# uta-smile/Adaptive-Graph-Convolutional-Network

Measured on NVIDIA B200. Metric: sgc_ll_train_graphs_per_s, higher is better.
Workload: dtype f32

## Files before the change

adaptive-graph-convolutional-network_b200/_lib.py:

```python
import ctypes
import os

HERE = os.path.dirname(os.path.abspath(__file__))
LIB_PATH = os.path.join(HERE, "libagcn_sm100.so")

AGCN_OK = 0
VARIANT = {"SGC_LL": 0, "SGC_LL_Reslap": 1}
LAPLACIAN = {"reference_literal": 0, "paper": 1}
METRIC_GRAD = {"reference": 0, "full": 1}
ACT = {"linear": 0, "relu": 1}
LOSS = {"sigmoid_ce": 0, "softmax_ce": 1}
ADJ_RULE = {"mean_distance": 0, "cutoff": 1}
NOTIFY_FN = ctypes.CFUNCTYPE(None, ctypes.c_void_p, ctypes.c_int32, ctypes.c_void_p)
OUT_RES_L, OUT_RES_W, OUT_L_ALL, SAVE_FOR_BACKWARD = 1, 2, 4, 8


class AgcnError(RuntimeError):
    pass


class Desc(ctypes.Structure):
    _fields_ = [("F", ctypes.c_int32), ("Fo", ctypes.c_int32), ("K", ctypes.c_int32), ("variant", ctypes.c_int32),
                ("laplacian_mode", ctypes.c_int32), ("metric_grad", ctypes.c_int32), ("activation", ctypes.c_int32),
                ("flags", ctypes.c_uint32)]
# ... 17 lines not shown
    "agcn_profile_enable": (ctypes.c_int, [ctypes.c_int]),
    "agcn_profile_read": (ctypes.c_int, [ctypes.c_char_p, ctypes.c_size_t, ctypes.POINTER(ctypes.c_size_t)]),
    "agcn_profile_timeline": (ctypes.c_int, [ctypes.c_char_p, ctypes.c_size_t, ctypes.POINTER(ctypes.c_size_t)]),
    "agcn_probe_fp32_fma": (ctypes.c_int, [_P, ctypes.c_int32, _P]),
    "agcn_pack_nodes": (ctypes.c_int, [_P, _P, _P, ctypes.c_int32, _P]),
    "agcn_unpack_nodes": (ctypes.c_int, [_P, _P, _P, ctypes.c_int32, _P]),
    "agcn_pack_lap": (ctypes.c_int, [_P, _P, _P, _P]),
    "agcn_capture_begin": (ctypes.c_int, [_P]),
    "agcn_capture_end_launch": (ctypes.c_int, [_P, ctypes.POINTER(ctypes.c_void_p), ctypes.POINTER(ctypes.c_int32)]),
    "agcn_capture_abort": (ctypes.c_int, [_P]),
    "agcn_step_graph_destroy": (ctypes.c_int, [_P]),
    "agcn_unpack_lap": (ctypes.c_int, [_P, _P, _P, _P]),
    "agcn_debug_grouped_product": (ctypes.c_int, [_P, _P, _P, _P, ctypes.c_int32, ctypes.c_int32, ctypes.c_int32,
                                                  ctypes.c_float, ctypes.c_int32, _P]),
    "agcn_debug_grouped_timeline": (ctypes.c_int, [_P]),
    "agcn_pack_lap_csr": (ctypes.c_int, [_P, _P, _P, _P, _P, _P]),
    "agcn_point_laplacian_workspace_bytes": (ctypes.c_int, [_P, ctypes.POINTER(ctypes.c_size_t)]),
    "agcn_point_laplacian": (ctypes.c_int, [_P, _P, ctypes.c_int32, ctypes.c_int32, ctypes.c_float, _P, _P,
                                            ctypes.c_size_t, _P]),
    "agcn_graph_pool": (ctypes.c_int, [_P, _P, _P, _P, _P, ctypes.c_int32, _P]),
    "agcn_graph_pool_backward": (ctypes.c_int, [_P, _P, _P, _P, ctypes.c_int32, _P]),
    "agcn_sgcll_workspace_bytes": (ctypes.c_int, [ctypes.POINTER(Desc), _P, ctypes.POINTER(ctypes.c_size_t),
                                                  ctypes.POINTER(ctypes.c_size_t)]),
    "agcn_sgcll_forward": (ctypes.c_int, [ctypes.POINTER(Desc), _P] + [_P] * 14 + [ctypes.c_size_t, _P]),
    "agcn_sgcll_backward": (ctypes.c_int, [ctypes.POINTER(Desc), _P] + [_P] * 19 + [ctypes.c_size_t, _P]),
    "agcn_gemm_tn_scratch_bytes": (ctypes.c_size_t, [ctypes.c_int32] * 4),
    "agcn_gemm_tn": (ctypes.c_int, [_P, _P, _P, _P, ctypes.c_int32, ctypes.c_int32, ctypes.c_int32, ctypes.c_int32,
                                    _P, ctypes.c_int32, _P]),
    "agcn_node_gemm_scratch_bytes": (ctypes.c_size_t, [ctypes.c_int32, ctypes.c_int32]),
    "agcn_node_gemm": (ctypes.c_int, [_P, ctypes.c_int32, _P, ctypes.c_int32, ctypes.c_int32, _P, ctypes.c_int32,
# ... 70 lines not shown
```

adaptive-graph-convolutional-network_b200/csrc/agcn_head.cu:

```cuda
#include <algorithm>

#include "agcn_internal.cuh"

namespace agcn {

__global__ void segment_sum_kernel(const float* __restrict__ H, const int32_t* __restrict__ node_off, int B, int F,
                                   float* __restrict__ hsum) {
  const int g = blockIdx.x * (blockDim.x >> 5) + (threadIdx.x >> 5), lane = threadIdx.x & 31;
  if (g >= B) return;
  const int r0 = node_off[g], r1 = node_off[g + 1];
  if (F % 32 == 0) {
    for (int c = lane; c < F; c += 32) {
      float s0 = 0.f, s1 = 0.f, s2 = 0.f, s3 = 0.f;
      int r = r0;
      for (; r + 4 <= r1; r += 4) {
        s0 += __ldg(H + (int64_t)r * F + c);
        s1 += __ldg(H + (int64_t)(r + 1) * F + c);
        s2 += __ldg(H + (int64_t)(r + 2) * F + c);
        s3 += __ldg(H + (int64_t)(r + 3) * F + c);
      }
      for (; r < r1; ++r) s0 += __ldg(H + (int64_t)r * F + c);
      hsum[(int64_t)g * F + c] = (s0 + s1) + (s2 + s3);
    }
    return;
// ... 26 lines not shown
  pre[e] = 4.f * ex / ((1.f + ex) * (1.f + ex));
}

__global__ void tanh_bwd_kernel(const float* __restrict__ dtanh, float* __restrict__ dmol, int64_t total) {
  const int64_t e = (int64_t)blockIdx.x * blockDim.x + threadIdx.x;
  if (e >= total) return;
  dmol[e] = dmol[e] * dtanh[e];
}

__global__ void __launch_bounds__(256) weighted_colsum_kernel(const float* __restrict__ M, int ld, int rows, int cols,
                                                              const int32_t* __restrict__ w, float* __restrict__ out) {
  __shared__ float red[8][33];
  const int lane = threadIdx.x & 31, wid = threadIdx.x >> 5;
  const int c = blockIdx.x * 32 + lane;
  float s = 0.f;
  if (c < cols)
    for (int r = wid; r < rows; r += 8) s += (w ? (float)w[r] : 1.f) * M[(int64_t)r * ld + c];
  red[wid][lane] = s;
  __syncthreads();
  if (wid == 0 && c < cols) {
    float t = 0.f;
#pragma unroll
    for (int k = 0; k < 8; ++k) t += red[k][lane];
    out[c] = t;
  }
}

__global__ void segment_broadcast_kernel(const float* __restrict__ dhsum, const int32_t* __restrict__ node_off, int B,
                                         int F, float* __restrict__ dH) {
  const int g = blockIdx.x * (blockDim.x >> 5) + (threadIdx.x >> 5), lane = threadIdx.x & 31;
  if (g >= B) return;
  const int r0 = node_off[g], r1 = node_off[g + 1];
  for (int c = lane; c < F; c += 32) {
    const float v = dhsum[(int64_t)g * F + c];
    for (int r = r0; r < r1; ++r) dH[(int64_t)r * F + c] = v;
  }
}

__global__ void copy_pitched_kernel(const float* __restrict__ src, int lds, float* __restrict__ dst, int ldd, int rows,
                                    int cols) {
  const int64_t e = (int64_t)blockIdx.x * blockDim.x + threadIdx.x;
  if (e >= (int64_t)rows * cols) return;
  const int r = (int)(e / cols), c = (int)(e % cols);
  dst[(int64_t)r * ldd + c] = src[(int64_t)r * lds + c];
}

__global__ void softmax_ce_kernel(float* __restrict__ logits, int ld, const float* __restrict__ y, const float* __restrict__ w,
                                  int B, int C, float scale, float* __restrict__ part) {
  const int b = blockIdx.x * (blockDim.x >> 5) + (threadIdx.x >> 5), lane = threadIdx.x & 31;
  if (b >= B) return;
  float* x = logits + (int64_t)b * ld;
  const float* yb = y + (int64_t)b * C;
  float mx = -INFINITY;
  for (int c = lane; c < C; c += 32) mx = fmaxf(mx, x[c]);
#pragma unroll
  for (int o = 16; o > 0; o >>= 1) mx = fmaxf(mx, __shfl_xor_sync(0xffffffffu, mx, o));
  float se = 0.f, sy = 0.f, sxy = 0.f;
  for (int c = lane; c < C; c += 32) {
    se += expf(x[c] - mx);
// ... 25 lines not shown
}

namespace {

int tn_any(const GemmTNArgs& t, cudaStream_t st) {
  if (tc_gemm_tn_supported(t)) return tc_gemm_tn(t, st);
  return gemm_tn(t, st);
}
size_t tn_any_partial(const GemmTNArgs& t) {
  return std::max(tc_gemm_tn_partial_floats(t), gemm_tn_partial_floats(t.M, t.Kd, t.N, t.S));
}

inline size_t al256(size_t x) { return (x + 255) & ~(size_t)255; }
inline int pad4(int x) { return (x + 3) & ~3; }

struct HeadWork {
  float *hsum, *pre, *mol, *dlog, *dmol, *dhsum, *dWh_pad, *loss_part, *tcA, *tcB, *tcC, *tcD, *tn_part, *splitk;
  size_t bytes;
};

HeadWork carve_head(const agcn_plan* plan, int Fh, int Fm, int Nt, void* base) {
  char* b = reinterpret_cast<char*>(base);
  size_t off = 0;
  auto take = [&](size_t floats) {
    float* r = b ? reinterpret_cast<float*>(b + off) : nullptr;
    off += al256(floats * sizeof(float));
    return r;
  };
  const size_t B = plan->B;
  const int Ntp = pad4(Nt);
  HeadWork w{};
  w.hsum = take(B * Fh);
// ... 5 lines not shown
  w.dWh_pad = take((size_t)Fm * Ntp);
  GemmArgs g;
  g.M = (int)B; g.N = Nt; g.Z = 1;
  w.loss_part = take(std::max((size_t)tc_gemm_loss_parts(g), B) + 64);
  w.tcA = take(tc_gemm_scratch_floats(Fm, Fh, 1, 1));
  w.tcB = take(tc_gemm_scratch_floats(Nt, Fm, 1, 1));
  w.tcC = take(tc_gemm_scratch_floats(Fm, Nt, 1, 1));
  w.tcD = take(tc_gemm_scratch_floats(Fh, Fm, 1, 1));
  GemmTNArgs t;
  t.M = (int)B; t.Kd = std::min(Fm, 128); t.N = Ntp; t.S = 1;
  size_t tn = tn_any_partial(t);
  t.Kd = Fh; t.N = Fm;
  tn = std::max(tn, tn_any_partial(t));
  w.tn_part = take(tn);
  w.splitk = take((size_t)8 * B * std::max(Fm, Fh));
  w.bytes = off;
  return w;
}

}
}

using namespace agcn;

extern "C" {

int agcn_expand_labels(const uint8_t* y, const float* w, int32_t B, int32_t n_tasks, float* d_targets, float* d_weights,
                       void* stream) {
  AGCN_REQUIRE(y && w && d_targets && d_weights && B >= 1 && n_tasks >= 1, "expand_labels: bad arguments");
  AGCN_REQUIRE((reinterpret_cast<uintptr_t>(d_targets) & 7) == 0 && (reinterpret_cast<uintptr_t>(d_weights) & 7) == 0,
               "expand_labels: outputs must be 8-byte aligned");
  const long long n = (long long)B * n_tasks;
  const unsigned grid = (unsigned)std::max<long long>(1, std::min<long long>((n + 1023) / 1024, 8));
  expand_labels_kernel<<<grid, 1024, 0, (cudaStream_t)stream>>>(y, w, n, reinterpret_cast<float2*>(d_targets),
                                                               reinterpret_cast<float2*>(d_weights));
  AGCN_LAUNCH_CHECK();
  return AGCN_OK;
}

int agcn_head_workspace_bytes(const agcn_plan* plan, int32_t Fh, int32_t Fm, int32_t Nt, size_t* bytes) {
  AGCN_REQUIRE(plan && bytes && Fh >= 1 && Fm >= 1 && Nt >= 1, "head_workspace_bytes: bad arguments");
  *bytes = carve_head(plan, Fh, Fm, Nt, nullptr).bytes + 256;
  return AGCN_OK;
}

int agcn_head_loss_grad(const agcn_plan* plan, const float* d_H, const float* d_dense_W, const float* d_dense_b,
                        const float* d_head_W, const float* d_head_b, const float* d_targets, const float* d_weights,
                        float scale, int32_t Fh, int32_t Fm, int32_t Nt, float* d_loss, float* d_dH,
                        float* d_ddense_W, float* d_ddense_b, float* d_dhead_W, float* d_dhead_b, void* d_work,
                        size_t work_bytes, void* stream) {
  return agcn_head_loss_grad_ex(plan, d_H, d_dense_W, d_dense_b, d_head_W, d_head_b, d_targets, d_weights, scale,
                                AGCN_LOSS_SIGMOID_CE, Fh, Fm, Nt, d_loss, d_dH, d_ddense_W, d_ddense_b, d_dhead_W,
                                d_dhead_b, d_work, work_bytes, stream);
}

int agcn_head_loss_grad_ex(const agcn_plan* plan, const float* d_H, const float* d_dense_W, const float* d_dense_b,
                           const float* d_head_W, const float* d_head_b, const float* d_targets, const float* d_weights,
                           float scale, int32_t loss_kind, int32_t Fh, int32_t Fm, int32_t Nt, float* d_loss,
                           float* d_dH, float* d_ddense_W, float* d_ddense_b, float* d_dhead_W, float* d_dhead_b,
                           void* d_work, size_t work_bytes, void* stream) {
  AGCN_REQUIRE(plan && d_H && d_dense_W && d_dense_b && d_head_W && d_head_b && d_targets && d_weights && d_loss &&
                   d_dH && d_ddense_W && d_ddense_b && d_dhead_W && d_dhead_b && d_work,
               "head_loss_grad: null pointer");
  AGCN_REQUIRE(loss_kind == AGCN_LOSS_SIGMOID_CE || loss_kind == AGCN_LOSS_SOFTMAX_CE, "head_loss_grad: unknown loss_kind");
  AGCN_REQUIRE(Fh >= 1 && Fm >= 32 && Fm % 4 == 0 && Nt >= 1,
               "head_loss_grad: unsupported sizes (need Fm >= 32 and a multiple of 4)");
  cudaStream_t st = (cudaStream_t)stream;
  int rc = plan_use(plan, st);
  if (rc) return rc;
  HeadWork w = carve_head(plan, Fh, Fm, Nt, d_work);
  if (w.bytes > work_bytes) {
    set_error("head_loss_grad: workspace too small");
    return AGCN_ERR_WORKSPACE;
  }
  const int B = plan->B, Ntp = pad4(Nt);
  const int R = (int)plan->R;
  (void)R;
  cudaStream_t side = plan->side;

  GemmArgs g_pre, g_log, g_dmol, g_dhs;
  g_pre.M = B; g_pre.N = Fm; g_pre.Kd = Fh;
  g_pre.A0 = w.hsum; g_pre.lda0 = Fh;
  g_pre.B = d_dense_W; g_pre.ldb = Fm;
  g_pre.C = w.pre; g_pre.ldc = Fm;
  g_log.M = B; g_log.N = Nt; g_log.Kd = Fm;
  g_log.A0 = w.mol; g_log.lda0 = Fm;
  g_log.B = d_head_W; g_log.ldb = Nt;
  g_log.C = w.dlog; g_log.ldc = Ntp;
  g_log.bias = d_head_b;
  const bool sigmoid = loss_kind == AGCN_LOSS_SIGMOID_CE;
  if (sigmoid) {
    g_log.bce_y = d_targets; g_log.bce_w = d_weights; g_log.bce_ld = Nt; g_log.bce_scale = scale;
    g_log.loss_part = w.loss_part;
  }
  g_dmol.M = B; g_dmol.N = Fm; g_dmol.Kd = Nt;
  g_dmol.A0 = w.dlog; g_dmol.lda0 = Ntp;
  g_dmol.B = d_head_W; g_dmol.ldb = Nt; g_dmol.transB = 1;
  g_dmol.C = w.dmol; g_dmol.ldc = Fm; g_dmol.split_k_partial = w.splitk;
  g_dhs.M = B; g_dhs.N = Fh; g_dhs.Kd = Fm;
  g_dhs.A0 = w.dmol; g_dhs.lda0 = Fm;
  g_dhs.B = d_dense_W; g_dhs.ldb = Fm; g_dhs.transB = 1;
  g_dhs.C = w.dhsum; g_dhs.ldc = Fh; g_dhs.split_k_partial = w.splitk;
  AGCN_REQUIRE(tc_gemm_supported(g_log), "head_loss_grad: operands are not TMA-compatible (alignment)");
  const bool tc_pre = false, tc_dmol = tc_gemm_supported(g_dmol), tc_dhs = tc_gemm_supported(g_dhs) && (int64_t)B * Fh * Fm > (1ll << 26);
  auto gemm_any = [&](const GemmArgs& g, const float* scratch, bool tc) { return tc ? tc_gemm(g, scratch, st) : gemm_rows(g, st); };
  AGCN_CUDA(cudaEventRecord(plan->ev_side_fork, st));
  AGCN_CUDA(cudaStreamWaitEvent(side, plan->ev_side_fork, 0));
  if (tc_pre && (rc = tc_gemm_split_b(g_pre, w.tcA, side))) return rc;
  if ((rc = tc_gemm_split_b(g_log, w.tcB, side))) return rc;
  if (tc_dmol && (rc = tc_gemm_split_b(g_dmol, w.tcC, side))) return rc;
  if (tc_dhs && (rc = tc_gemm_split_b(g_dhs, w.tcD, side))) return rc;
  if ((rc = zero_async(w.dlog, (size_t)B * Ntp, side))) return rc;
  AGCN_CUDA(cudaEventRecord(plan->ev_side_join, side));

  segment_sum_kernel<<<(B + 7) / 8, 256, 0, st>>>(d_H, plan->d_node_off, B, Fh, w.hsum);
  AGCN_LAUNCH_CHECK();
  AGCN_CUDA(cudaStreamWaitEvent(st, plan->ev_side_join, 0));
  if ((rc = gemm_any(g_pre, w.tcA, tc_pre))) return rc;
  {
    const int64_t total = (int64_t)B * Fm;
    gather_tanh_kernel<<<(unsigned)((total + 255) / 256), 256, 0, st>>>(w.pre, d_dense_b, plan->d_n, B, Fm, w.mol);
    AGCN_LAUNCH_CHECK();
  }
  if ((rc = tc_gemm(g_log, w.tcB, st))) return rc;
  int n_parts = tc_gemm_loss_parts(g_log);
  if (!sigmoid) {
    softmax_ce_kernel<<<(B + 7) / 8, 256, 0, st>>>(w.dlog, Ntp, d_targets, d_weights, B, Nt, scale, w.loss_part);
    AGCN_LAUNCH_CHECK();
    n_parts = B;
  }
  sum_parts_kernel<<<1, 256, 0, st>>>(w.loss_part, n_parts, d_loss);
  AGCN_LAUNCH_CHECK();

  AGCN_CUDA(cudaEventRecord(plan->ev_side_fork, st));
  AGCN_CUDA(cudaStreamWaitEvent(side, plan->ev_side_fork, 0));
  weighted_colsum_kernel<<<(Nt + 31) / 32, 256, 0, side>>>(w.dlog, Ntp, B, Nt, nullptr, d_dhead_b);
  AGCN_LAUNCH_CHECK();
  for (int f0 = 0; f0 < Fm; f0 += 128) {
    GemmTNArgs t;
    t.M = B; t.Kd = std::min(128, Fm - f0); t.N = Ntp; t.S = 1;
    t.A0 = w.mol + f0; t.lda0 = Fm;
    t.D = w.dlog; t.ldd = Ntp;
    t.out = w.dWh_pad + (size_t)f0 * Ntp; t.partial = w.tn_part;
    if ((rc = tn_any(t, side))) return rc;
  }
  {
    const int64_t total = (int64_t)Fm * Nt;
    copy_pitched_kernel<<<(unsigned)((total + 255) / 256), 256, 0, side>>>(w.dWh_pad, Ntp, d_dhead_W, Nt, Fm, Nt);
    AGCN_LAUNCH_CHECK();
  }

  if ((rc = gemm_any(g_dmol, w.tcC, tc_dmol))) return rc;
  {
    const int64_t total = (int64_t)B * Fm;
    tanh_bwd_kernel<<<(unsigned)((total + 255) / 256), 256, 0, st>>>(w.pre, w.dmol, total);
    AGCN_LAUNCH_CHECK();
  }
  if ((rc = gemm_any(g_dhs, w.tcD, tc_dhs))) return rc;
  segment_broadcast_kernel<<<(B + 7) / 8, 256, 0, st>>>(w.dhsum, plan->d_node_off, B, Fh, d_dH);
  AGCN_LAUNCH_CHECK();
  AGCN_CUDA(cudaEventRecord(plan->ev_fork, st));
  AGCN_CUDA(cudaStreamWaitEvent(side, plan->ev_fork, 0));
  weighted_colsum_kernel<<<(Fm + 31) / 32, 256, 0, side>>>(w.dmol, Fm, B, Fm, plan->d_n, d_ddense_b);
  AGCN_LAUNCH_CHECK();
  {
    GemmTNArgs t;
    t.M = B; t.Kd = Fh; t.N = Fm; t.S = 1;
    t.A0 = w.hsum; t.lda0 = Fh;
    t.D = w.dmol; t.ldd = Fm;
    t.out = d_ddense_W; t.partial = w.tn_part;
    if ((rc = tn_any(t, side))) return rc;
  }
  AGCN_CUDA(cudaEventRecord(plan->ev_side_join, side));
  AGCN_CUDA(cudaStreamWaitEvent(st, plan->ev_side_join, 0));
  return AGCN_OK;
}

}
```

adaptive-graph-convolutional-network_b200/csrc/agcn_internal.cuh:

```cuda
#pragma once
#include <cuda_runtime.h>
#include <stdint.h>

#include <atomic>
#include <string>
#include <vector>

#include "agcn_sgcll.h"

#define AGCN_SMALL_MAX 144
#define AGCN_CHEB_SMALL_MAX 144
#define AGCN_FUSE_MAX_N 64
#define AGCN_FUSE_LCAP 8320
#define AGCN_MID_TILED_MIN 32
#define AGCN_DEGREE_FLOOR 8.271806125530277e-25f

namespace agcn {

#ifdef __CUDACC__
__device__ __forceinline__ float tf32_rn(float x) {
  uint32_t r;
  asm("cvt.rna.tf32.f32 %0, %1;\n" : "=r"(r) : "f"(x));
  return __uint_as_float(r);
}
// ... 118 lines not shown
  int64_t sliceB = 0;
  int transB = 0;
  float* C = nullptr;
  int ldc = 0;
  int64_t sliceC = 0;
  const float* bias = nullptr;
  const float* scale = nullptr;
  int act = AGCN_ACT_LINEAR;
  int accumulate = 0;
  const float* bce_y = nullptr;
  const float* bce_w = nullptr;
  int bce_ld = 0;
  float bce_scale = 1.f;
  float* loss_part = nullptr;
  float* split_k_partial = nullptr;
};
int tc_gemm_loss_parts(const GemmArgs& a);
int gemm_rows(const GemmArgs& a, cudaStream_t st);
bool tc_gemm_supported(const GemmArgs& a);
size_t tc_gemm_scratch_floats(int N, int Kd, int S, int Z);
int tc_gemm_split_b(const GemmArgs& a, float* scratch, cudaStream_t st);
int tc_gemm(const GemmArgs& a, const float* scratch, cudaStream_t st);

struct GemmTNArgs {
  int M = 0;
  int Kd = 0;
  int N = 0;
  int S = 1;
  const float* A0 = nullptr;
  int lda0 = 0;
  const float* A1 = nullptr;
  int lda1 = 0;
  int64_t sliceA1 = 0;
  const float* D = nullptr;
  int ldd = 0;
  float* out = nullptr;
  float* partial = nullptr;
// ... 106 lines not shown
                        cudaStream_t st_small, cudaStream_t st_mid);

class ProfScope {
 public:
  ProfScope(const char* name, cudaStream_t st);
  ~ProfScope();
  ProfScope(const ProfScope&) = delete;
  ProfScope& operator=(const ProfScope&) = delete;

 private:
  const char* name_;
  cudaStream_t st_;
  cudaEvent_t e0_;
};

int zero_async(float* dst, size_t floats, cudaStream_t st);
int plan_use(const agcn_plan* plan, cudaStream_t st);
int fork_streams(const agcn_plan* plan, cudaStream_t main, int n_aux);
int join_streams(const agcn_plan* plan, cudaStream_t main, int n_aux);

}
```

adaptive-graph-convolutional-network_b200/csrc/agcn_stack.cu:

```cuda
#include <algorithm>
#include <cmath>
#include <vector>

#include "agcn_internal.cuh"

struct agcn_stack {
  std::vector<agcn_sgcll_desc> layers;
  int32_t Fm = 0, Nt = 0, loss_kind = 0;
  std::vector<int64_t> off;
};

namespace agcn {

__global__ void __launch_bounds__(256) adam_kernel(float* __restrict__ p, const float* __restrict__ g, float* __restrict__ m,
                                                   float* __restrict__ v, const int32_t* __restrict__ step, long long n,
                                                   float lr, float beta1, float beta2, float eps) {
  __shared__ float s_lr_t;
  if (threadIdx.x == 0) {
    const double t = (double)(*step + 1);
    s_lr_t = (float)((double)lr * sqrt(1.0 - pow((double)beta2, t)) / (1.0 - pow((double)beta1, t)));
  }
  __syncthreads();
  const float lr_t = s_lr_t;
  for (long long i = (long long)blockIdx.x * blockDim.x + threadIdx.x; i < n; i += (long long)gridDim.x * blockDim.x) {
// ... 109 lines not shown
    return AGCN_ERR_WORKSPACE;
  }
  const int nl = (int)s->layers.size();
  auto P = [&](int l, int k) { return s->off[5 * (size_t)l + k] >= 0 ? d_params + s->off[5 * (size_t)l + k] : nullptr; };
  auto G = [&](int l, int k) { return s->off[5 * (size_t)l + k] >= 0 ? d_grads + s->off[5 * (size_t)l + k] : nullptr; };
  const int64_t* ho = &s->off[5 * (size_t)nl];
  const float* x = d_X;
  for (int l = 0; l < nl; ++l) {
    const agcn_sgcll_desc& d = s->layers[l];
    rc = agcn_sgcll_forward(&d, plan, x, d_Lint, nullptr, P(l, 2), P(l, 0), P(l, 1), P(l, 3), nullptr, w.H[l], nullptr,
                            nullptr, nullptr, w.saved[l], w.layer_work, w.layer_work_bytes, stream);
    if (rc) return rc;
    x = w.H[l];
  }
  const agcn_sgcll_desc& last = s->layers[nl - 1];
  rc = agcn_head_loss_grad_ex(plan, w.H[nl - 1], d_params + ho[0], d_params + ho[1], d_params + ho[2], d_params + ho[3],
                              d_targets, d_weights, scale, s->loss_kind, last.Fo, s->Fm, s->Nt, d_loss, w.dA,
                              d_grads + ho[0], d_grads + ho[1], d_grads + ho[2], d_grads + ho[3], w.head_work,
                              w.head_work_bytes, stream);
  if (rc) return rc;
  if (notify) notify(notify_user, nl, stream);
  float* dcur = w.dA;
  float* dnext = w.dB;
  for (int l = nl - 1; l >= 0; --l) {
    const agcn_sgcll_desc& d = s->layers[l];
    const bool full = d.laplacian_mode == AGCN_LAP_PAPER && d.metric_grad == AGCN_METRIC_GRAD_FULL;
    float* dX = (l > 0 || full) ? dnext : nullptr;
    rc = agcn_sgcll_backward(&d, plan, l == 0 ? d_X : w.H[l - 1], d_Lint, nullptr, P(l, 2), P(l, 0), P(l, 3), nullptr,
                             w.H[l], dcur, nullptr, w.saved[l], dX, G(l, 2), G(l, 0), G(l, 1), G(l, 3), nullptr, nullptr,
                             w.layer_work, w.layer_work_bytes, stream);
    if (rc) return rc;
    if (notify) notify(notify_user, l, stream);
    std::swap(dcur, dnext);
  }
// ... 104 lines not shown
```

adaptive-graph-convolutional-network_b200/csrc/agcn_tc_gemm.cu:

```cuda
#include <cuda.h>
#include <cstdio>

#include <algorithm>
#include <cstdlib>
#include <mutex>

#include "agcn_internal.cuh"

namespace agcn {

namespace tc {

constexpr int BM = 128;
constexpr int BK = 32;
constexpr int UMMA_K = 8;
constexpr int A_TILE_BYTES = BM * BK * 4;

__device__ __forceinline__ uint32_t smem_u32(const void* p) { return (uint32_t)__cvta_generic_to_shared(p); }

__device__ __forceinline__ void mbar_init(uint64_t* bar, uint32_t count) {
  asm volatile("mbarrier.init.shared::cta.b64 [%0], %1;\n" ::"r"(smem_u32(bar)), "r"(count) : "memory");
}
__device__ __forceinline__ void mbar_expect_tx(uint64_t* bar, uint32_t bytes) {
  asm volatile("mbarrier.arrive.expect_tx.shared::cta.b64 _, [%0], %1;\n" ::"r"(smem_u32(bar)), "r"(bytes) : "memory");
// ... 577 lines not shown
  return true;
}

static bool tc_gemm_narrow2(const GemmArgs& a) {
  const int Npad = tc_npad(a.N);
  if (!a.bce_y || Npad <= 64) return false;
  const int tiles128 = ((a.M + tc::BM - 1) / tc::BM) * a.Z * (Npad / 128);
  return tiles128 < 148;
}

int tc_gemm_loss_parts(const GemmArgs& a) {
  const int Npad = tc_npad(a.N), BN = (Npad <= 64 || tc_gemm_narrow2(a)) ? 64 : 128;
  return 4 * ((a.M + tc::BM - 1) / tc::BM) * a.Z * (Npad / BN);
}

size_t tc_gemm_scratch_floats(int N, int Kd, int S, int Z) { return 2 * (size_t)Z * S * tc_npad(N) * tc_kpitch(Kd); }

int tc_gemm_split_b(const GemmArgs& a, float* scratch, cudaStream_t st) {
  using namespace tc;
  const long long sn = a.transB ? a.ldb : 1, sk = a.transB ? 1 : a.ldb, ss = a.sliceB;
  const int Npad = tc_npad(a.N), Kp = tc_kpitch(a.Kd);
  const int slices = a.Z * a.S;
  float* Bhi = scratch;
  float* Blo = scratch + (size_t)slices * Npad * Kp;
  const long long total = (long long)slices * Npad * Kp;
  const int blocks = (int)std::min<long long>((total + 255) / 256, 1184);
  split_b_kernel<<<blocks, 256, 0, st>>>(a.B, sn, sk, ss, a.N, Npad, a.Kd, Kp, slices, Bhi, Blo);
  AGCN_LAUNCH_CHECK();
  return AGCN_OK;
}
// ... 10 lines not shown
  const int rows_slice1 = a.S > 1 ? (int)(a.sliceA1 / a.lda1) : 0;
  if (a.S > 1) {
    if ((rc = make_map(&mA1, a.A1, (uint64_t)(a.S - 2) * rows_slice1 + a.M, (uint64_t)a.Kd, (uint64_t)a.lda1, BM)))
      return rc;
  } else {
    mA1 = mA0;
  }
  const bool narrow2 = tc_gemm_narrow2(a);
  const int BN = (Npad <= 64 || narrow2) ? 64 : 128;
  if ((rc = make_map(&mBhi, Bhi, (uint64_t)slices * Npad, (uint64_t)a.Kd, (uint64_t)Kp, BN))) return rc;
  if ((rc = make_map(&mBlo, Blo, (uint64_t)slices * Npad, (uint64_t)a.Kd, (uint64_t)Kp, BN))) return rc;
  Args p;
  p.M = a.M; p.N = a.N; p.Kd = a.Kd; p.S = a.S;
  p.kb_per_slice = (a.Kd + BK - 1) / BK;
  const int total_kb = a.S * p.kb_per_slice;
  const int out_tiles = ((a.M + BM - 1) / BM) * a.Z * (Npad / BN);
  int ksplit = 1;
  if (a.split_k_partial && !a.bias && !a.scale && a.act == AGCN_ACT_LINEAR && !a.accumulate && !a.bce_y && a.ldc == a.N && a.Z == 1 &&
      total_kb >= 16 && out_tiles < 74)
    ksplit = std::min(std::min(8, total_kb / 4), std::max(1, 148 / out_tiles));
  p.ksplit = ksplit;
  p.kb_per_split = (total_kb + ksplit - 1) / ksplit;
  p.ksplit = (total_kb + p.kb_per_split - 1) / p.kb_per_split;
  ksplit = p.ksplit;
  p.rows_slice1 = rows_slice1;
  p.b_rows_slice = Npad;
  p.C = a.C; p.ldc = a.ldc; p.sliceC = a.sliceC;
  if (ksplit > 1) {
    p.C = a.split_k_partial;
    p.sliceC = (long long)a.M * a.ldc;
  }
  p.bias = a.bias; p.scale = a.scale; p.act = a.act; p.accumulate = a.accumulate;
  p.bce_y = a.bce_y; p.bce_w = a.bce_w; p.bce_scale = a.bce_scale; p.loss_part = a.loss_part;
  p.bce_ld = a.bce_ld > 0 ? a.bce_ld : a.ldc;
  dim3 grid((a.M + BM - 1) / BM, a.Z * ksplit, Npad / BN);
  static std::once_flag once64, once128;
  if (narrow2) {
    static std::once_flag once642;
    std::call_once(once642, [] {
// ... 9 lines not shown
    });
    {
      ProfScope prof("tc::tc_gemm_kernel", st);
      tc_gemm_kernel<64><<<grid, 192, Smem<64>::TOTAL, st>>>(mA0, mA1, mBhi, mBlo, p);
    }
  } else {
    std::call_once(once128, [] {
      cudaFuncSetAttribute(tc_gemm_kernel<128>, cudaFuncAttributeMaxDynamicSharedMemorySize, Smem<128>::TOTAL);
    });
    {
      ProfScope prof("tc::tc_gemm_kernel", st);
      tc_gemm_kernel<128><<<grid, 192, Smem<128>::TOTAL, st>>>(mA0, mA1, mBhi, mBlo, p);
    }
  }
  AGCN_LAUNCH_CHECK();
  if (ksplit > 1) {
    const long long elems = (long long)a.M * a.ldc;
    reduce_chunks_kernel<<<(unsigned)((elems + 255) / 256), 256, 0, st>>>(a.split_k_partial, a.C, elems, ksplit);
    AGCN_LAUNCH_CHECK();
  }
  return AGCN_OK;
}

}

namespace agcn {

bool tc_gemm_tn_supported(const GemmTNArgs& a) {
  if (ab_env("AGCN_DISABLE_TCGEN05") || ab_env("AGCN_DISABLE_TCGEN05_TN")) return false;
  auto al16 = [](const void* p) { return (reinterpret_cast<uintptr_t>(p) & 15) == 0; };
  if (a.M < 32 || a.Kd > 128 || a.Kd % 4 != 0 || a.N % 4 != 0) return false;
// ... 77 lines not shown
```

include/agcn_sgcll.h:

```cpp
#ifndef AGCN_SGCLL_H_
#define AGCN_SGCLL_H_

#include <stdint.h>
#include <stddef.h>

#ifdef __cplusplus
extern "C" {
#endif

#define AGCN_OK 0
#define AGCN_ERR_INVALID (-1)
#define AGCN_ERR_CUDA (-2)
#define AGCN_ERR_WORKSPACE (-3)
#define AGCN_ERR_NO_DEVICE (-4)

#define AGCN_VARIANT_SGC_LL 0
#define AGCN_VARIANT_SGC_LL_RESLAP 1
#define AGCN_LAP_REFERENCE_LITERAL 0
#define AGCN_LAP_PAPER 1
#define AGCN_METRIC_GRAD_REFERENCE 0
#define AGCN_METRIC_GRAD_FULL 1
#define AGCN_ACT_LINEAR 0
#define AGCN_ACT_RELU 1

// ... 32 lines not shown
int agcn_fused_profile(int enable);
int agcn_fused_profile_read(float* ms_sum, int* launches);

int agcn_profile_enable(int enable);
int agcn_profile_read(char* buf, size_t cap, size_t* needed);
int agcn_profile_timeline(char* buf, size_t cap, size_t* needed);
int agcn_probe_fp32_fma(float* d_sink, int32_t iters, void* stream);

int agcn_fused_debug_set(void* d_buf);

int agcn_debug_grouped_product(const agcn_plan* plan, const float* d_L , const float* d_In ,
                               float* d_Out , int32_t F, int32_t transL, int32_t add_identity, float cmul,
                               int32_t impl, void* stream);

int agcn_debug_grouped_timeline(void* d_buf);

int agcn_pack_nodes(const agcn_plan* plan, const float* d_padded , float* d_packed ,
                    int32_t F, void* stream);
int agcn_unpack_nodes(const agcn_plan* plan, const float* d_packed, float* d_padded, int32_t F, void* stream);
int agcn_pack_lap(const agcn_plan* plan, const float* d_padded , float* d_packed, void* stream);
int agcn_unpack_lap(const agcn_plan* plan, const float* d_packed, float* d_padded, void* stream);
int agcn_pack_lap_csr(const agcn_plan* plan, const int32_t* d_indptr, const int32_t* d_indices, const float* d_values,
                      float* d_packed, void* stream);

#define AGCN_ADJ_MEAN_DISTANCE 0
#define AGCN_ADJ_CUTOFF 1
int agcn_point_laplacian_workspace_bytes(const agcn_plan* plan, size_t* bytes);
int agcn_point_laplacian(const agcn_plan* plan, const float* d_points, int32_t F, int32_t rule, float sparse_ratio,
                         float* d_L, void* d_work, size_t work_bytes, void* stream);

// ... 81 lines not shown
```

Measured before the change: 1.648 million.

## Fuse head segment-sum, dense GEMM and tanh into gather kernels with deferred split-k

Adds fused head kernels. The forward kernel does the per-graph segment sum, the dense projection and tanh plus its derivative in one pass. The backward kernel does the split-k reduction, the tanh backward, the dH-sum GEMM against a transposed weight and the broadcast to nodes. The goal is fewer kernel launches and fewer intermediate round trips through global memory in the small-batch head. It also moves sum_parts to the side stream and adds a weight transpose on that stream. The cost is that the GEMMs run on CUDA cores instead of tensor cores, with a shared-memory limit guard and an env or debug switch to fall back to the old path.

```diff
diff --git a/adaptive-graph-convolutional-network_b200/_lib.py b/adaptive-graph-convolutional-network_b200/_lib.py
--- a/adaptive-graph-convolutional-network_b200/_lib.py
+++ b/adaptive-graph-convolutional-network_b200/_lib.py
@@ -55,6 +55,7 @@
     "agcn_debug_grouped_product": (ctypes.c_int, [_P, _P, _P, _P, ctypes.c_int32, ctypes.c_int32, ctypes.c_int32,
                                                   ctypes.c_float, ctypes.c_int32, _P]),
     "agcn_debug_grouped_timeline": (ctypes.c_int, [_P]),
+    "agcn_debug_head_path": (ctypes.c_int, [ctypes.c_int32]),
     "agcn_pack_lap_csr": (ctypes.c_int, [_P, _P, _P, _P, _P, _P]),
     "agcn_point_laplacian_workspace_bytes": (ctypes.c_int, [_P, ctypes.POINTER(ctypes.c_size_t)]),
     "agcn_point_laplacian": (ctypes.c_int, [_P, _P, ctypes.c_int32, ctypes.c_int32, ctypes.c_float, _P, _P,
diff --git a/adaptive-graph-convolutional-network_b200/csrc/agcn_head.cu b/adaptive-graph-convolutional-network_b200/csrc/agcn_head.cu
--- a/adaptive-graph-convolutional-network_b200/csrc/agcn_head.cu
+++ b/adaptive-graph-convolutional-network_b200/csrc/agcn_head.cu
@@ -1,4 +1,5 @@
 #include <algorithm>
+#include <atomic>
 
 #include "agcn_internal.cuh"
 
@@ -64,8 +65,10 @@
   const int lane = threadIdx.x & 31, wid = threadIdx.x >> 5;
   const int c = blockIdx.x * 32 + lane;
   float s = 0.f;
-  if (c < cols)
+  if (c < cols) {
+#pragma unroll 8
     for (int r = wid; r < rows; r += 8) s += (w ? (float)w[r] : 1.f) * M[(int64_t)r * ld + c];
+  }
   red[wid][lane] = s;
   __syncthreads();
   if (wid == 0 && c < cols) {
@@ -87,12 +90,132 @@
   }
 }
 
+__global__ void transpose_kernel(const float* __restrict__ src, int rows, int cols, float* __restrict__ dst) {
+  const int64_t e = (int64_t)blockIdx.x * blockDim.x + threadIdx.x;
+  if (e >= (int64_t)rows * cols) return;
+  const int r = (int)(e / cols), c = (int)(e % cols);
+  dst[(int64_t)c * rows + r] = src[e];
+}
+
 __global__ void copy_pitched_kernel(const float* __restrict__ src, int lds, float* __restrict__ dst, int ldd, int rows,
                                     int cols) {
   const int64_t e = (int64_t)blockIdx.x * blockDim.x + threadIdx.x;
   if (e >= (int64_t)rows * cols) return;
   const int r = (int)(e / cols), c = (int)(e % cols);
   dst[(int64_t)r * ldd + c] = src[(int64_t)r * lds + c];
+}
+
+constexpr int HEAD_G = 8;
+constexpr int HEAD_KC = 16;
+
+
+__global__ void __launch_bounds__(256) head_gather_fwd_kernel(const float* __restrict__ H, const int32_t* __restrict__ node_off,
+                                                              const int32_t* __restrict__ n_nodes, const float* __restrict__ Wd,
+                                                              const float* __restrict__ bd, int B, int Fh, int Fm, int G,
+                                                              float* __restrict__ hsum, float* __restrict__ dtanh,
+                                                              float* __restrict__ mol) {
+  extern __shared__ __align__(16) float hs[];
+  const int g0 = blockIdx.x * G, ng = min(G, B - g0);
+  for (int e = threadIdx.x; e < ng * Fh; e += blockDim.x) {
+    const int gi = e / Fh, c = e - gi * Fh;
+    const int r0 = node_off[g0 + gi], r1 = node_off[g0 + gi + 1];
+    float v;
+    if (Fh % 32 == 0) {
+      float s0 = 0.f, s1 = 0.f, s2 = 0.f, s3 = 0.f;
+      int r = r0;
+      for (; r + 4 <= r1; r += 4) {
+        s0 += __ldg(H + (int64_t)r * Fh + c);
+        s1 += __ldg(H + (int64_t)(r + 1) * Fh + c);
+        s2 += __ldg(H + (int64_t)(r + 2) * Fh + c);
+        s3 += __ldg(H + (int64_t)(r + 3) * Fh + c);
+      }
+      for (; r < r1; ++r) s0 += __ldg(H + (int64_t)r * Fh + c);
+      v = (s0 + s1) + (s2 + s3);
+    } else {
+      v = 0.f;
+      for (int r = r0; r < r1; ++r) v += H[(int64_t)r * Fh + c];
+    }
+    hs[e] = v;
+    hsum[(int64_t)g0 * Fh + e] = v;
+  }
+  __syncthreads();
+  for (int j = threadIdx.x; j < Fm; j += blockDim.x) {
+    float acc[HEAD_G];
+#pragma unroll
+    for (int gi = 0; gi < HEAD_G; ++gi) acc[gi] = 0.f;
+    for (int k = 0; k < Fh; k += 4) {
+      const float w0 = __ldg(Wd + (int64_t)k * Fm + j), w1 = __ldg(Wd + (int64_t)(k + 1) * Fm + j);
+      const float w2 = __ldg(Wd + (int64_t)(k + 2) * Fm + j), w3 = __ldg(Wd + (int64_t)(k + 3) * Fm + j);
+#pragma unroll
+      for (int gi = 0; gi < HEAD_G; ++gi)
+        if (gi < ng) {
+          const float4 a = *reinterpret_cast<const float4*>(hs + gi * Fh + k);
+          acc[gi] += a.x * w0 + a.y * w1 + a.z * w2 + a.w * w3;
+        }
+    }
+    const float bj = bd[j];
+#pragma unroll
+    for (int gi = 0; gi < HEAD_G; ++gi) {
+      if (gi >= ng) break;
+      const int64_t e = (int64_t)(g0 + gi) * Fm + j;
+      const float a = acc[gi] + (float)n_nodes[g0 + gi] * bj;
+      mol[e] = tanhf(a);
+      const float ex = expf(-2.f * fabsf(a));
+      dtanh[e] = 4.f * ex / ((1.f + ex) * (1.f + ex));
+    }
+  }
+}
+
+__global__ void __launch_bounds__(256) head_gather_bwd_kernel(const float* dmol, int nsplit, int64_t split_stride,
+                                                              const float* __restrict__ dtanh, const float* __restrict__ WdT,
+                                                              const int32_t* __restrict__ node_off, int B, int Fh, int Fm,
+                                                              int G, float* dpre, float* __restrict__ dH) {
+  extern __shared__ __align__(16) float sm[];
+  const int g0 = blockIdx.x * G, ng = min(G, B - g0);
+  float* dp = sm;
+  float* dhs = sm + ng * Fm;
+  for (int e = threadIdx.x; e < ng * Fm; e += blockDim.x) {
+    const int64_t idx = (int64_t)g0 * Fm + e;
+    float s = 0.f;
+    for (int z = 0; z < nsplit; ++z) s += dmol[z * split_stride + idx];
+    const float v = s * dtanh[idx];
+    dp[e] = v;
+    dpre[idx] = v;
+  }
+  __syncthreads();
+  float* ws = dhs + ng * Fh;
+  float acc[8];
+#pragma unroll
+  for (int i = 0; i < 8; ++i) acc[i] = 0.f;
+  for (int k0 = 0; k0 < Fm; k0 += HEAD_KC) {
+    const int kc = min(HEAD_KC, Fm - k0);
+    __syncthreads();
+    for (int e = threadIdx.x; e < kc * Fh; e += blockDim.x) ws[e] = __ldg(WdT + (int64_t)k0 * Fh + e);
+    __syncthreads();
+#pragma unroll
+    for (int i = 0; i < 8; ++i) {
+      const int e = threadIdx.x + i * blockDim.x;
+      if (e < ng * Fh) {
+        const int gi = e / Fh, c = e - gi * Fh;
+        for (int k = 0; k < kc; k += 4) {
+          const float4 a = *reinterpret_cast<const float4*>(dp + gi * Fm + k0 + k);
+          acc[i] += a.x * ws[k * Fh + c] + a.y * ws[(k + 1) * Fh + c] + a.z * ws[(k + 2) * Fh + c] +
+                    a.w * ws[(k + 3) * Fh + c];
+        }
+      }
+    }
+  }
+#pragma unroll
+  for (int i = 0; i < 8; ++i) {
+    const int e = threadIdx.x + i * blockDim.x;
+    if (e < ng * Fh) dhs[e] = acc[i];
+  }
+  __syncthreads();
+  for (int gi = 0; gi < ng; ++gi) {
+    const int r0 = node_off[g0 + gi], r1 = node_off[g0 + gi + 1];
+    float* out = dH + (int64_t)r0 * Fh;
+    for (int e = threadIdx.x; e < (r1 - r0) * Fh; e += blockDim.x) out[e] = dhs[gi * Fh + e % Fh];
+  }
 }
 
 __global__ void softmax_ce_kernel(float* __restrict__ logits, int ld, const float* __restrict__ y, const float* __restrict__ w,
@@ -148,8 +271,20 @@
 inline size_t al256(size_t x) { return (x + 255) & ~(size_t)255; }
 inline int pad4(int x) { return (x + 3) & ~3; }
 
+std::atomic<int> g_head_unfused{0};
+
+inline int head_graphs_per_cta(int B) { return std::min(HEAD_G, std::max(1, (B + 147) / 148)); }
+
+bool head_fused(int B, int Fh, int Fm) {
+  if (g_head_unfused.load(std::memory_order_relaxed) || ab_env("AGCN_HEAD_UNFUSED")) return false;
+  if (Fh % 4 != 0 || Fh > 256) return false;
+  const size_t G = (size_t)head_graphs_per_cta(B);
+  return (G * (Fm + Fh) + HEAD_KC * Fh) * sizeof(float) <= 48 * 1024;
+}
+
 struct HeadWork {
   float *hsum, *pre, *mol, *dlog, *dmol, *dhsum, *dWh_pad, *loss_part, *tcA, *tcB, *tcC, *tcD, *tn_part, *splitk;
+  float* dense_WT;
   size_t bytes;
 };
 
@@ -185,58 +320,24 @@
   tn = std::max(tn, tn_any_partial(t));
   w.tn_part = take(tn);
   w.splitk = take((size_t)8 * B * std::max(Fm, Fh));
+  w.dense_WT = take((size_t)Fh * Fm);
   w.bytes = off;
   return w;
 }
 
 }
-}
-
-using namespace agcn;
-
-extern "C" {
-
-int agcn_expand_labels(const uint8_t* y, const float* w, int32_t B, int32_t n_tasks, float* d_targets, float* d_weights,
-                       void* stream) {
-  AGCN_REQUIRE(y && w && d_targets && d_weights && B >= 1 && n_tasks >= 1, "expand_labels: bad arguments");
-  AGCN_REQUIRE((reinterpret_cast<uintptr_t>(d_targets) & 7) == 0 && (reinterpret_cast<uintptr_t>(d_weights) & 7) == 0,
-               "expand_labels: outputs must be 8-byte aligned");
-  const long long n = (long long)B * n_tasks;
-  const unsigned grid = (unsigned)std::max<long long>(1, std::min<long long>((n + 1023) / 1024, 8));
-  expand_labels_kernel<<<grid, 1024, 0, (cudaStream_t)stream>>>(y, w, n, reinterpret_cast<float2*>(d_targets),
-                                                               reinterpret_cast<float2*>(d_weights));
-  AGCN_LAUNCH_CHECK();
-  return AGCN_OK;
-}
-
-int agcn_head_workspace_bytes(const agcn_plan* plan, int32_t Fh, int32_t Fm, int32_t Nt, size_t* bytes) {
-  AGCN_REQUIRE(plan && bytes && Fh >= 1 && Fm >= 1 && Nt >= 1, "head_workspace_bytes: bad arguments");
-  *bytes = carve_head(plan, Fh, Fm, Nt, nullptr).bytes + 256;
-  return AGCN_OK;
-}
-
-int agcn_head_loss_grad(const agcn_plan* plan, const float* d_H, const float* d_dense_W, const float* d_dense_b,
-                        const float* d_head_W, const float* d_head_b, const float* d_targets, const float* d_weights,
-                        float scale, int32_t Fh, int32_t Fm, int32_t Nt, float* d_loss, float* d_dH,
-                        float* d_ddense_W, float* d_ddense_b, float* d_dhead_W, float* d_dhead_b, void* d_work,
-                        size_t work_bytes, void* stream) {
-  return agcn_head_loss_grad_ex(plan, d_H, d_dense_W, d_dense_b, d_head_W, d_head_b, d_targets, d_weights, scale,
-                                AGCN_LOSS_SIGMOID_CE, Fh, Fm, Nt, d_loss, d_dH, d_ddense_W, d_ddense_b, d_dhead_W,
-                                d_dhead_b, d_work, work_bytes, stream);
-}
-
-int agcn_head_loss_grad_ex(const agcn_plan* plan, const float* d_H, const float* d_dense_W, const float* d_dense_b,
-                           const float* d_head_W, const float* d_head_b, const float* d_targets, const float* d_weights,
-                           float scale, int32_t loss_kind, int32_t Fh, int32_t Fm, int32_t Nt, float* d_loss,
-                           float* d_dH, float* d_ddense_W, float* d_ddense_b, float* d_dhead_W, float* d_dhead_b,
-                           void* d_work, size_t work_bytes, void* stream) {
+
+int head_loss_grad(const agcn_plan* plan, const float* d_H, const float* d_dense_W, const float* d_dense_b,
+                   const float* d_head_W, const float* d_head_b, const float* d_targets, const float* d_weights, float scale,
+                   int32_t loss_kind, int32_t Fh, int32_t Fm, int32_t Nt, float* d_loss, float* d_dH, float* d_ddense_W,
+                   float* d_ddense_b, float* d_dhead_W, float* d_dhead_b, void* d_work, size_t work_bytes, bool join,
+                   cudaStream_t st) {
   AGCN_REQUIRE(plan && d_H && d_dense_W && d_dense_b && d_head_W && d_head_b && d_targets && d_weights && d_loss &&
                    d_dH && d_ddense_W && d_ddense_b && d_dhead_W && d_dhead_b && d_work,
                "head_loss_grad: null pointer");
   AGCN_REQUIRE(loss_kind == AGCN_LOSS_SIGMOID_CE || loss_kind == AGCN_LOSS_SOFTMAX_CE, "head_loss_grad: unknown loss_kind");
   AGCN_REQUIRE(Fh >= 1 && Fm >= 32 && Fm % 4 == 0 && Nt >= 1,
                "head_loss_grad: unsupported sizes (need Fm >= 32 and a multiple of 4)");
-  cudaStream_t st = (cudaStream_t)stream;
   int rc = plan_use(plan, st);
   if (rc) return rc;
   HeadWork w = carve_head(plan, Fh, Fm, Nt, d_work);
@@ -245,9 +346,9 @@
     return AGCN_ERR_WORKSPACE;
   }
   const int B = plan->B, Ntp = pad4(Nt);
-  const int R = (int)plan->R;
-  (void)R;
   cudaStream_t side = plan->side;
+  const bool fused = head_fused(B, Fh, Fm);
+  const int G = head_graphs_per_cta(B), n_cta = (B + G - 1) / G;
 
   GemmArgs g_pre, g_log, g_dmol, g_dhs;
   g_pre.M = B; g_pre.N = Fm; g_pre.Kd = Fh;
@@ -268,12 +369,14 @@
   g_dmol.A0 = w.dlog; g_dmol.lda0 = Ntp;
   g_dmol.B = d_head_W; g_dmol.ldb = Nt; g_dmol.transB = 1;
   g_dmol.C = w.dmol; g_dmol.ldc = Fm; g_dmol.split_k_partial = w.splitk;
+  g_dmol.split_k_defer = fused ? 1 : 0;
   g_dhs.M = B; g_dhs.N = Fh; g_dhs.Kd = Fm;
   g_dhs.A0 = w.dmol; g_dhs.lda0 = Fm;
   g_dhs.B = d_dense_W; g_dhs.ldb = Fm; g_dhs.transB = 1;
   g_dhs.C = w.dhsum; g_dhs.ldc = Fh; g_dhs.split_k_partial = w.splitk;
   AGCN_REQUIRE(tc_gemm_supported(g_log), "head_loss_grad: operands are not TMA-compatible (alignment)");
-  const bool tc_pre = false, tc_dmol = tc_gemm_supported(g_dmol), tc_dhs = tc_gemm_supported(g_dhs) && (int64_t)B * Fh * Fm > (1ll << 26);
+  const bool tc_pre = false, tc_dmol = tc_gemm_supported(g_dmol);
+  const bool tc_dhs = !fused && tc_gemm_supported(g_dhs) && (int64_t)B * Fh * Fm > (1ll << 26);
   auto gemm_any = [&](const GemmArgs& g, const float* scratch, bool tc) { return tc ? tc_gemm(g, scratch, st) : gemm_rows(g, st); };
   AGCN_CUDA(cudaEventRecord(plan->ev_side_fork, st));
   AGCN_CUDA(cudaStreamWaitEvent(side, plan->ev_side_fork, 0));
@@ -282,30 +385,58 @@
   if (tc_dmol && (rc = tc_gemm_split_b(g_dmol, w.tcC, side))) return rc;
   if (tc_dhs && (rc = tc_gemm_split_b(g_dhs, w.tcD, side))) return rc;
   if ((rc = zero_async(w.dlog, (size_t)B * Ntp, side))) return rc;
+  if (fused) {
+    const int64_t total = (int64_t)Fh * Fm;
+    transpose_kernel<<<(unsigned)((total + 255) / 256), 256, 0, side>>>(d_dense_W, Fh, Fm, w.dense_WT);
+    AGCN_LAUNCH_CHECK();
+  }
   AGCN_CUDA(cudaEventRecord(plan->ev_side_join, side));
 
-  segment_sum_kernel<<<(B + 7) / 8, 256, 0, st>>>(d_H, plan->d_node_off, B, Fh, w.hsum);
-  AGCN_LAUNCH_CHECK();
-  AGCN_CUDA(cudaStreamWaitEvent(st, plan->ev_side_join, 0));
-  if ((rc = gemm_any(g_pre, w.tcA, tc_pre))) return rc;
-  {
+  if (fused) {
+    {
+      ProfScope prof("head::head_gather_fwd_kernel", st);
+      head_gather_fwd_kernel<<<n_cta, 256, (size_t)G * Fh * sizeof(float), st>>>(
+          d_H, plan->d_node_off, plan->d_n, d_dense_W, d_dense_b, B, Fh, Fm, G, w.hsum, w.pre, w.mol);
+    }
+    AGCN_LAUNCH_CHECK();
+    AGCN_CUDA(cudaStreamWaitEvent(st, plan->ev_side_join, 0));
+  } else {
+    {
+      ProfScope prof("head::segment_sum_kernel", st);
+      segment_sum_kernel<<<(B + 7) / 8, 256, 0, st>>>(d_H, plan->d_node_off, B, Fh, w.hsum);
+    }
+    AGCN_LAUNCH_CHECK();
+    AGCN_CUDA(cudaStreamWaitEvent(st, plan->ev_side_join, 0));
+    if ((rc = gemm_any(g_pre, w.tcA, tc_pre))) return rc;
     const int64_t total = (int64_t)B * Fm;
-    gather_tanh_kernel<<<(unsigned)((total + 255) / 256), 256, 0, st>>>(w.pre, d_dense_b, plan->d_n, B, Fm, w.mol);
+    {
+      ProfScope prof("head::gather_tanh_kernel", st);
+      gather_tanh_kernel<<<(unsigned)((total + 255) / 256), 256, 0, st>>>(w.pre, d_dense_b, plan->d_n, B, Fm, w.mol);
+    }
     AGCN_LAUNCH_CHECK();
   }
   if ((rc = tc_gemm(g_log, w.tcB, st))) return rc;
   int n_parts = tc_gemm_loss_parts(g_log);
   if (!sigmoid) {
-    softmax_ce_kernel<<<(B + 7) / 8, 256, 0, st>>>(w.dlog, Ntp, d_targets, d_weights, B, Nt, scale, w.loss_part);
+    {
+      ProfScope prof("head::softmax_ce_kernel", st);
+      softmax_ce_kernel<<<(B + 7) / 8, 256, 0, st>>>(w.dlog, Ntp, d_targets, d_weights, B, Nt, scale, w.loss_part);
+    }
     AGCN_LAUNCH_CHECK();
     n_parts = B;
   }
-  sum_parts_kernel<<<1, 256, 0, st>>>(w.loss_part, n_parts, d_loss);
-  AGCN_LAUNCH_CHECK();
 
   AGCN_CUDA(cudaEventRecord(plan->ev_side_fork, st));
   AGCN_CUDA(cudaStreamWaitEvent(side, plan->ev_side_fork, 0));
-  weighted_colsum_kernel<<<(Nt + 31) / 32, 256, 0, side>>>(w.dlog, Ntp, B, Nt, nullptr, d_dhead_b);
+  {
+    ProfScope prof("head::sum_parts_kernel", side);
+    sum_parts_kernel<<<1, 256, 0, side>>>(w.loss_part, n_parts, d_loss);
+  }
+  AGCN_LAUNCH_CHECK();
+  {
+    ProfScope prof("head::weighted_colsum_kernel", side);
+    weighted_colsum_kernel<<<(Nt + 31) / 32, 256, 0, side>>>(w.dlog, Ntp, B, Nt, nullptr, d_dhead_b);
+  }
   AGCN_LAUNCH_CHECK();
   for (int f0 = 0; f0 < Fm; f0 += 128) {
     GemmTNArgs t;
@@ -322,17 +453,35 @@
   }
 
   if ((rc = gemm_any(g_dmol, w.tcC, tc_dmol))) return rc;
-  {
+  if (fused) {
+    const int nsplit = tc_dmol ? tc_gemm_ksplit(g_dmol) : 1;
+    const float* src = nsplit > 1 ? w.splitk : w.dmol;
+    {
+      ProfScope prof("head::head_gather_bwd_kernel", st);
+      head_gather_bwd_kernel<<<n_cta, 256, ((size_t)G * (Fm + Fh) + HEAD_KC * Fh) * sizeof(float), st>>>(
+          src, nsplit, (int64_t)B * Fm, w.pre, w.dense_WT, plan->d_node_off, B, Fh, Fm, G, w.dmol, d_dH);
+    }
+    AGCN_LAUNCH_CHECK();
+  } else {
     const int64_t total = (int64_t)B * Fm;
-    tanh_bwd_kernel<<<(unsigned)((total + 255) / 256), 256, 0, st>>>(w.pre, w.dmol, total);
-    AGCN_LAUNCH_CHECK();
-  }
-  if ((rc = gemm_any(g_dhs, w.tcD, tc_dhs))) return rc;
-  segment_broadcast_kernel<<<(B + 7) / 8, 256, 0, st>>>(w.dhsum, plan->d_node_off, B, Fh, d_dH);
-  AGCN_LAUNCH_CHECK();
+    {
+      ProfScope prof("head::tanh_bwd_kernel", st);
+      tanh_bwd_kernel<<<(unsigned)((total + 255) / 256), 256, 0, st>>>(w.pre, w.dmol, total);
+    }
+    AGCN_LAUNCH_CHECK();
+    if ((rc = gemm_any(g_dhs, w.tcD, tc_dhs))) return rc;
+    {
+      ProfScope prof("head::segment_broadcast_kernel", st);
+      segment_broadcast_kernel<<<(B + 7) / 8, 256, 0, st>>>(w.dhsum, plan->d_node_off, B, Fh, d_dH);
+    }
+    AGCN_LAUNCH_CHECK();
+  }
   AGCN_CUDA(cudaEventRecord(plan->ev_fork, st));
   AGCN_CUDA(cudaStreamWaitEvent(side, plan->ev_fork, 0));
-  weighted_colsum_kernel<<<(Fm + 31) / 32, 256, 0, side>>>(w.dmol, Fm, B, Fm, plan->d_n, d_ddense_b);
+  {
+    ProfScope prof("head::weighted_colsum_kernel", side);
+    weighted_colsum_kernel<<<(Fm + 31) / 32, 256, 0, side>>>(w.dmol, Fm, B, Fm, plan->d_n, d_ddense_b);
+  }
   AGCN_LAUNCH_CHECK();
   {
     GemmTNArgs t;
@@ -343,8 +492,58 @@
     if ((rc = tn_any(t, side))) return rc;
   }
   AGCN_CUDA(cudaEventRecord(plan->ev_side_join, side));
-  AGCN_CUDA(cudaStreamWaitEvent(st, plan->ev_side_join, 0));
+  if (join) AGCN_CUDA(cudaStreamWaitEvent(st, plan->ev_side_join, 0));
   return AGCN_OK;
 }
 
 }
+
+using namespace agcn;
+
+extern "C" {
+
+int agcn_expand_labels(const uint8_t* y, const float* w, int32_t B, int32_t n_tasks, float* d_targets, float* d_weights,
+                       void* stream) {
+  AGCN_REQUIRE(y && w && d_targets && d_weights && B >= 1 && n_tasks >= 1, "expand_labels: bad arguments");
+  AGCN_REQUIRE((reinterpret_cast<uintptr_t>(d_targets) & 7) == 0 && (reinterpret_cast<uintptr_t>(d_weights) & 7) == 0,
+               "expand_labels: outputs must be 8-byte aligned");
+  const long long n = (long long)B * n_tasks;
+  const unsigned grid = (unsigned)std::max<long long>(1, std::min<long long>((n + 1023) / 1024, 8));
+  expand_labels_kernel<<<grid, 1024, 0, (cudaStream_t)stream>>>(y, w, n, reinterpret_cast<float2*>(d_targets),
+                                                               reinterpret_cast<float2*>(d_weights));
+  AGCN_LAUNCH_CHECK();
+  return AGCN_OK;
+}
+
+int agcn_head_workspace_bytes(const agcn_plan* plan, int32_t Fh, int32_t Fm, int32_t Nt, size_t* bytes) {
+  AGCN_REQUIRE(plan && bytes && Fh >= 1 && Fm >= 1 && Nt >= 1, "head_workspace_bytes: bad arguments");
+  *bytes = carve_head(plan, Fh, Fm, Nt, nullptr).bytes + 256;
+  return AGCN_OK;
+}
+
+int agcn_head_loss_grad(const agcn_plan* plan, const float* d_H, const float* d_dense_W, const float* d_dense_b,
+                        const float* d_head_W, const float* d_head_b, const float* d_targets, const float* d_weights,
+                        float scale, int32_t Fh, int32_t Fm, int32_t Nt, float* d_loss, float* d_dH,
+                        float* d_ddense_W, float* d_ddense_b, float* d_dhead_W, float* d_dhead_b, void* d_work,
+                        size_t work_bytes, void* stream) {
+  return agcn_head_loss_grad_ex(plan, d_H, d_dense_W, d_dense_b, d_head_W, d_head_b, d_targets, d_weights, scale,
+                                AGCN_LOSS_SIGMOID_CE, Fh, Fm, Nt, d_loss, d_dH, d_ddense_W, d_ddense_b, d_dhead_W,
+                                d_dhead_b, d_work, work_bytes, stream);
+}
+
+int agcn_head_loss_grad_ex(const agcn_plan* plan, const float* d_H, const float* d_dense_W, const float* d_dense_b,
+                           const float* d_head_W, const float* d_head_b, const float* d_targets, const float* d_weights,
+                           float scale, int32_t loss_kind, int32_t Fh, int32_t Fm, int32_t Nt, float* d_loss,
+                           float* d_dH, float* d_ddense_W, float* d_ddense_b, float* d_dhead_W, float* d_dhead_b,
+                           void* d_work, size_t work_bytes, void* stream) {
+  return head_loss_grad(plan, d_H, d_dense_W, d_dense_b, d_head_W, d_head_b, d_targets, d_weights, scale, loss_kind, Fh,
+                        Fm, Nt, d_loss, d_dH, d_ddense_W, d_ddense_b, d_dhead_W, d_dhead_b, d_work, work_bytes,
+                        true, (cudaStream_t)stream);
+}
+
+int agcn_debug_head_path(int32_t unfused) {
+  g_head_unfused.store(unfused ? 1 : 0);
+  return AGCN_OK;
+}
+
+}
diff --git a/adaptive-graph-convolutional-network_b200/csrc/agcn_internal.cuh b/adaptive-graph-convolutional-network_b200/csrc/agcn_internal.cuh
--- a/adaptive-graph-convolutional-network_b200/csrc/agcn_internal.cuh
+++ b/adaptive-graph-convolutional-network_b200/csrc/agcn_internal.cuh
@@ -156,6 +156,7 @@
   float bce_scale = 1.f;
   float* loss_part = nullptr;
   float* split_k_partial = nullptr;
+  int split_k_defer = 0;
 };
 int tc_gemm_loss_parts(const GemmArgs& a);
 int gemm_rows(const GemmArgs& a, cudaStream_t st);
@@ -163,6 +164,7 @@
 size_t tc_gemm_scratch_floats(int N, int Kd, int S, int Z);
 int tc_gemm_split_b(const GemmArgs& a, float* scratch, cudaStream_t st);
 int tc_gemm(const GemmArgs& a, const float* scratch, cudaStream_t st);
+int tc_gemm_ksplit(const GemmArgs& a);
 
 struct GemmTNArgs {
   int M = 0;
@@ -299,6 +301,12 @@
   cudaEvent_t e0_;
 };
 
+int head_loss_grad(const agcn_plan* plan, const float* d_H, const float* d_dense_W, const float* d_dense_b,
+                   const float* d_head_W, const float* d_head_b, const float* d_targets, const float* d_weights, float scale,
+                   int32_t loss_kind, int32_t Fh, int32_t Fm, int32_t Nt, float* d_loss, float* d_dH, float* d_ddense_W,
+                   float* d_ddense_b, float* d_dhead_W, float* d_dhead_b, void* d_work, size_t work_bytes, bool join,
+                   cudaStream_t st);
+
 int zero_async(float* dst, size_t floats, cudaStream_t st);
 int plan_use(const agcn_plan* plan, cudaStream_t st);
 int fork_streams(const agcn_plan* plan, cudaStream_t main, int n_aux);
diff --git a/adaptive-graph-convolutional-network_b200/csrc/agcn_stack.cu b/adaptive-graph-convolutional-network_b200/csrc/agcn_stack.cu
--- a/adaptive-graph-convolutional-network_b200/csrc/agcn_stack.cu
+++ b/adaptive-graph-convolutional-network_b200/csrc/agcn_stack.cu
@@ -147,10 +147,10 @@
     x = w.H[l];
   }
   const agcn_sgcll_desc& last = s->layers[nl - 1];
-  rc = agcn_head_loss_grad_ex(plan, w.H[nl - 1], d_params + ho[0], d_params + ho[1], d_params + ho[2], d_params + ho[3],
-                              d_targets, d_weights, scale, s->loss_kind, last.Fo, s->Fm, s->Nt, d_loss, w.dA,
-                              d_grads + ho[0], d_grads + ho[1], d_grads + ho[2], d_grads + ho[3], w.head_work,
-                              w.head_work_bytes, stream);
+  rc = head_loss_grad(plan, w.H[nl - 1], d_params + ho[0], d_params + ho[1], d_params + ho[2], d_params + ho[3], d_targets,
+                      d_weights, scale, s->loss_kind, last.Fo, s->Fm, s->Nt, d_loss, w.dA, d_grads + ho[0], d_grads + ho[1],
+                      d_grads + ho[2], d_grads + ho[3], w.head_work, w.head_work_bytes, notify != nullptr,
+                      (cudaStream_t)stream);
   if (rc) return rc;
   if (notify) notify(notify_user, nl, stream);
   float* dcur = w.dA;
diff --git a/adaptive-graph-convolutional-network_b200/csrc/agcn_tc_gemm.cu b/adaptive-graph-convolutional-network_b200/csrc/agcn_tc_gemm.cu
--- a/adaptive-graph-convolutional-network_b200/csrc/agcn_tc_gemm.cu
+++ b/adaptive-graph-convolutional-network_b200/csrc/agcn_tc_gemm.cu
@@ -615,6 +615,20 @@
   return 4 * ((a.M + tc::BM - 1) / tc::BM) * a.Z * (Npad / BN);
 }
 
+int tc_gemm_ksplit(const GemmArgs& a) {
+  using namespace tc;
+  const int Npad = tc_npad(a.N);
+  const int BN = (Npad <= 64 || tc_gemm_narrow2(a)) ? 64 : 128;
+  const int total_kb = a.S * ((a.Kd + BK - 1) / BK);
+  const int out_tiles = ((a.M + BM - 1) / BM) * a.Z * (Npad / BN);
+  int ksplit = 1;
+  if (a.split_k_partial && !a.bias && !a.scale && a.act == AGCN_ACT_LINEAR && !a.accumulate && !a.bce_y && a.ldc == a.N && a.Z == 1 &&
+      total_kb >= 16 && out_tiles < 74)
+    ksplit = std::min(std::min(8, total_kb / 4), std::max(1, 148 / out_tiles));
+  const int per = (total_kb + ksplit - 1) / ksplit;
+  return (total_kb + per - 1) / per;
+}
+
 size_t tc_gemm_scratch_floats(int N, int Kd, int S, int Z) { return 2 * (size_t)Z * S * tc_npad(N) * tc_kpitch(Kd); }
 
 int tc_gemm_split_b(const GemmArgs& a, float* scratch, cudaStream_t st) {
@@ -655,15 +669,9 @@
   p.M = a.M; p.N = a.N; p.Kd = a.Kd; p.S = a.S;
   p.kb_per_slice = (a.Kd + BK - 1) / BK;
   const int total_kb = a.S * p.kb_per_slice;
-  const int out_tiles = ((a.M + BM - 1) / BM) * a.Z * (Npad / BN);
-  int ksplit = 1;
-  if (a.split_k_partial && !a.bias && !a.scale && a.act == AGCN_ACT_LINEAR && !a.accumulate && !a.bce_y && a.ldc == a.N && a.Z == 1 &&
-      total_kb >= 16 && out_tiles < 74)
-    ksplit = std::min(std::min(8, total_kb / 4), std::max(1, 148 / out_tiles));
+  int ksplit = tc_gemm_ksplit(a);
+  p.kb_per_split = (total_kb + ksplit - 1) / ksplit;
   p.ksplit = ksplit;
-  p.kb_per_split = (total_kb + ksplit - 1) / ksplit;
-  p.ksplit = (total_kb + p.kb_per_split - 1) / p.kb_per_split;
-  ksplit = p.ksplit;
   p.rows_slice1 = rows_slice1;
   p.b_rows_slice = Npad;
   p.C = a.C; p.ldc = a.ldc; p.sliceC = a.sliceC;
@@ -703,7 +711,7 @@
     }
   }
   AGCN_LAUNCH_CHECK();
-  if (ksplit > 1) {
+  if (ksplit > 1 && !a.split_k_defer) {
     const long long elems = (long long)a.M * a.ldc;
     reduce_chunks_kernel<<<(unsigned)((elems + 255) / 256), 256, 0, st>>>(a.split_k_partial, a.C, elems, ksplit);
     AGCN_LAUNCH_CHECK();
diff --git a/include/agcn_sgcll.h b/include/agcn_sgcll.h
--- a/include/agcn_sgcll.h
+++ b/include/agcn_sgcll.h
@@ -70,6 +70,8 @@
                                int32_t impl, void* stream);
 
 int agcn_debug_grouped_timeline(void* d_buf);
+
+int agcn_debug_head_path(int32_t unfused);
 
 int agcn_pack_nodes(const agcn_plan* plan, const float* d_padded , float* d_packed ,
                     int32_t F, void* stream);
```

Measured after the change: 1.715 million (median of 6 runs). 1.04x the previous value.
